# amolrpatil21/PorQua

Hardware: AMD Instinct MI355X
Metric: QPs solved/sec (rebalance dates) at N=1000 assets, 1-8 GPU; x vs host CPU (higher is better)
Workload: dtype f64; 1 GPU; config3: long-only min-variance (P=2*Pearson cov, budget + box [0,1]), daily rebalance; n_assets=1000, window=252, dates_per_gpu=4749, global_batch=4749, parallelism=dates-sharded x1

## Files before the change

include/porqua_hip.h:

```cpp
#ifndef PORQUA_HIP_H
#define PORQUA_HIP_H

#include <stdint.h>

#ifdef __cplusplus
extern "C" {
#endif

#define PQ_VERSION 100

#define PQ_UNSOLVED 0
#define PQ_SOLVED 1
#define PQ_SOLVED_INACCURATE 2
#define PQ_MAX_ITER 3
#define PQ_NEED_REFACTOR 4
#define PQ_PRIMAL_INFEASIBLE (-3)
#define PQ_DUAL_INFEASIBLE (-4)
#define PQ_NON_CONVEX (-5)

#define PQ_OUT_OBJ 0
#define PQ_OUT_PRIM 1
#define PQ_OUT_DUAL 2
#define PQ_OUT_GAP 3
#define PQ_OUT_RHO 4
// ... 15 lines not shown
  const double* lb;  const double* ub;  int64_t box_stride;
} pq_problem;

typedef struct pq_state {
  double* K;     int64_t K_stride;
  double* Dt;    int64_t Dt_stride;
  double* x;     double* Px;
  double* z;     double* y;
  int32_t m_ld, mg_pad;
  double* rho;
  int32_t* iters; int32_t* status; int32_t* info;
  double* out;
  double* work;  int64_t work_stride;
} pq_state;

typedef struct pq_settings {
  double rho0, rho0_rel, sigma, alpha, eps_abs, eps_rel, rho_min, rho_max, adapt_tol, eq_scale,
      delta, dual_tol;
  int32_t max_iter, adapt_interval, polish, polish_rounds, refine_iters;
  double polish_fix_rel;
  int32_t polish_inner;
  int32_t min_iter;
  double polish_release_rel;
} pq_settings;

typedef struct pq_lowrank {
  const double* panel; int64_t ldp;
  const int32_t* rows; const int32_t* tlen; int32_t tmax;
  const double* mu; int64_t mu_stride;
  const double* w_scale;
  const double* dg; int64_t dg_stride;
} pq_lowrank;

int pq_version(void);
const char* pq_last_error(void);

int pq_window_mean(const double* panel, int64_t ldp, int32_t n, const int32_t* rows,
                   const int32_t* tlen, int32_t tmax, int32_t batch, double* mu,
                   int64_t mu_stride, void* stream);

int pq_window_sumsq(const double* panel, int64_t ldp, int32_t n, const int32_t* rows,
                    const int32_t* tlen, int32_t tmax, int32_t batch, const double* mu,
                    int64_t mu_stride, double* out, int64_t out_stride, void* stream);

int pq_window_moments_grouped(const double* panel, int64_t ldp, int32_t n, const int32_t* gdates,
                              int32_t ngroups, const int32_t* urows, int32_t umax,
// ... 238 lines not shown
```

porqua_amd/_lib.py:

```python
from __future__ import annotations

import ctypes
import os

_HERE = os.path.dirname(os.path.abspath(__file__))
LIB_PATH = os.environ.get("PQ_LIB_PATH") or os.path.join(_HERE, "libporqua_hip.so")

c_int32 = ctypes.c_int32
c_int64 = ctypes.c_int64
c_dp = ctypes.c_void_p

PQ_UNSOLVED = 0
PQ_SOLVED = 1
PQ_SOLVED_INACCURATE = 2
PQ_MAX_ITER = 3
PQ_NEED_REFACTOR = 4
PQ_PRIMAL_INFEASIBLE = -3
PQ_DUAL_INFEASIBLE = -4
PQ_NON_CONVEX = -5

PQ_PCT_OK, PQ_PCT_EMPTY_BUCKET, PQ_PCT_NAN_SCORE = range(3)
PQ_PCT_MAX_N = 16384
PQ_PCT_MAX_BUCKETS = 256

PQ_RP_OK, PQ_RP_MAX_SWEEPS, PQ_RP_BAD_INPUT = range(3)
PQ_RP_TMAX = 1024

PQ_HRP_OK, PQ_HRP_BAD_INPUT = range(2)
PQ_HRP_NMAX = 1024
PQ_HRP_SINGLE, PQ_HRP_COMPLETE, PQ_HRP_AVERAGE, PQ_HRP_WEIGHTED, PQ_HRP_WARD = range(5)
HRP_METHODS = {"single": PQ_HRP_SINGLE, "complete": PQ_HRP_COMPLETE, "average": PQ_HRP_AVERAGE,
               "weighted": PQ_HRP_WEIGHTED, "ward": PQ_HRP_WARD}

PQ_PCA_TMAX = 1024
PQ_PCA_KMAX = 64
PQ_PCA_OK, PQ_PCA_BAD_INPUT = range(2)

PQ_PG_RECORD = 384
PQ_PG_PASS_SCRATCH = 123537
PQ_PG_PENDING, PQ_PG_DONE, PQ_PG_FALLBACK, PQ_PG_SKIP = range(4)
PQ_PG_STATE = 3
PQ_PG_K, PQ_PG_SC, PQ_PG_W = 0, 5, 320

PQ_OUT_OBJ, PQ_OUT_PRIM, PQ_OUT_DUAL, PQ_OUT_GAP, PQ_OUT_RHO, PQ_OUT_NFREE, PQ_OUT_ROUNDS = range(7)
PQ_OUT_FIELDS = 8


def work_doubles(ld: int, mg_pad: int) -> int:
    return (9 + mg_pad) * ld + 512


class PorquaHipError(RuntimeError):
    pass


class PQProblem(ctypes.Structure):
    _fields_ = [
        ("n", c_int32), ("ld", c_int32), ("batch", c_int32), ("mg", c_int32),
        ("P", c_dp), ("P_stride", c_int64),
        ("p_scale", c_dp), ("p_diag", c_dp),
        ("q", c_dp), ("q_stride", c_int64),
        ("Cg", c_dp), ("Cg_stride", c_int64),
        ("lg", c_dp), ("ug", c_dp), ("g_stride", c_int64),
        ("lb", c_dp), ("ub", c_dp), ("box_stride", c_int64),
    ]
# ... 6 lines not shown
        ("x", c_dp), ("Px", c_dp),
        ("z", c_dp), ("y", c_dp),
        ("m_ld", c_int32), ("mg_pad", c_int32),
        ("rho", c_dp),
        ("iters", c_dp), ("status", c_dp), ("info", c_dp),
        ("out", c_dp),
        ("work", c_dp), ("work_stride", c_int64),
    ]


class PQSettings(ctypes.Structure):
    _fields_ = [
        ("rho0", ctypes.c_double), ("rho0_rel", ctypes.c_double),
        ("sigma", ctypes.c_double), ("alpha", ctypes.c_double),
        ("eps_abs", ctypes.c_double), ("eps_rel", ctypes.c_double),
        ("rho_min", ctypes.c_double), ("rho_max", ctypes.c_double),
        ("adapt_tol", ctypes.c_double), ("eq_scale", ctypes.c_double),
        ("delta", ctypes.c_double), ("dual_tol", ctypes.c_double),
        ("max_iter", c_int32), ("adapt_interval", c_int32), ("polish", c_int32),
        ("polish_rounds", c_int32), ("refine_iters", c_int32),
        ("polish_fix_rel", ctypes.c_double),
        ("polish_inner", ctypes.c_int32), ("min_iter", ctypes.c_int32),
        ("polish_release_rel", ctypes.c_double),
    ]


class PQLowRank(ctypes.Structure):
    _fields_ = [
        ("panel", c_dp), ("ldp", c_int64),
        ("rows", c_dp), ("tlen", c_dp), ("tmax", c_int32),
        ("mu", c_dp), ("mu_stride", c_int64),
        ("w_scale", c_dp),
        ("dg", c_dp), ("dg_stride", c_int64),
    ]


class PQGcap(ctypes.Structure):
    _fields_ = [
        ("gdates", c_dp), ("ngroups", c_int32),
        ("urows", c_dp), ("ucnt", c_dp), ("uoff", c_dp), ("umax", c_int32),
        ("gidx", c_dp), ("grho", c_dp),
        ("M", c_dp), ("Minv", c_dp), ("k_ld", c_int32), ("M_stride", c_int64),
        ("aq", c_dp), ("aq_stride", c_int64),
        ("hinv", c_dp), ("ldh", c_int32),
        ("gmax", c_int32),
    ]
# ... 157 lines not shown
```

porqua_amd/csrc/admm.hip:

```cpp
#include "admm_dev.h"
#include "capi_util.h"

namespace pq {

constexpr int AT = 512;
constexpr int AW = AT / 64;

struct PhaseClock {
#ifdef PQ_PROFILE
  long long a[8];
  long long t;
  __device__ void init() {
    for (int i = 0; i < 8; ++i) a[i] = 0;
    t = wall_clock64();
  }
  __device__ void stamp(int k) {
    __syncthreads();
    if (threadIdx.x == 0) {
      const long long now = wall_clock64();
      a[k] += now - t;
      t = now;
    }
  }
  __device__ void flush(double* dst) {
// ... 453 lines not shown
      gz[t] = zg[t];
      gy[t] = yg[t];
    }
    if (t == 0) {
      st.iters[b] = it;
      st.status[b] = status;
      st.rho[b] = rho;
    }
  }
}

__global__ void k_init_state(pq_problem pb, pq_state st, const int32_t* idx, pq_settings s,
                             const double* dg, int64_t dg_stride, const double* w_scale) {
  const int b = idx ? idx[blockIdx.x] : (int)blockIdx.x;
  const int ld = pb.ld;
  for (int i = threadIdx.x; i < ld; i += blockDim.x) {
    st.x[(int64_t)b * ld + i] = 0.0;
    st.Px[(int64_t)b * ld + i] = 0.0;
  }
  for (int i = threadIdx.x; i < st.m_ld; i += blockDim.x) {
    st.z[(int64_t)b * st.m_ld + i] = 0.0;
    st.y[(int64_t)b * st.m_ld + i] = 0.0;
  }
  double rho0 = s.rho0;
  if (s.rho0_rel > 0.0) {
    __shared__ double red[16];
    const double* P = pb.P + (int64_t)b * pb.P_stride;
    const double ps = pb.p_scale ? pb.p_scale[b] : 1.0;
    const double pd = pb.p_diag ? pb.p_diag[b] : 0.0;
    double sdiag = 0.0;
    if (dg) {
      const double psw = ps * (w_scale ? w_scale[b] : 1.0);
      for (int i = threadIdx.x; i < pb.n; i += blockDim.x) sdiag += psw * dg[(int64_t)b * dg_stride + i] + pd;
    } else {
      for (int i = threadIdx.x; i < pb.n; i += blockDim.x) sdiag += ps * P[(int64_t)i * ld + i] + pd;
    }
    sdiag = block_sum(sdiag, red);
    const double md = sdiag / pb.n;
    rho0 = (md > 0.0 && isfinite(md)) ? fmin(fmax(s.rho0_rel * md, s.rho_min), s.rho_max) : s.rho0;
  }
  if (threadIdx.x == 0) {
    st.rho[b] = rho0;
    st.iters[b] = 0;
    st.status[b] = PQ_UNSOLVED;
    st.info[b] = 0;
    for (int k = 0; k < PQ_OUT_FIELDS; ++k)
      st.out[(int64_t)b * PQ_OUT_FIELDS + k] = (k == PQ_OUT_OBJ || k == PQ_OUT_PRIM || k == PQ_OUT_DUAL ||
                                                k == PQ_OUT_GAP) ? __builtin_nan("") : 0.0;
  }
}

}

extern "C" int pq_init_state(const pq_problem* pb, pq_state* st, const int32_t* idx, int32_t nidx,
                             const pq_settings* s, void* stream) {
  PQ_CHECK_ARG(pb && st && s, "pq_init_state: null argument");
  PQ_CHECK_ARG(st->x && st->Px && st->z && st->y && st->rho && st->iters && st->status &&
                   st->info && st->out, "pq_init_state: state buffers missing");
  PQ_CHECK_ARG(st->m_ld >= st->mg_pad + pb->ld && st->mg_pad >= pb->mg, "pq_init_state: bad m_ld / mg_pad");
  const int grid = idx ? nidx : pb->batch;
  if (grid <= 0) return 0;
  PQ_CHECK_ARG(pb->P || s->rho0_rel <= 0.0, "pq_init_state: rho0_rel > 0 needs P (pq_init_state_lr for the window form)");
// ... 81 lines not shown
```

porqua_amd/csrc/admm_gcap.hip:

```cpp
#include "admm_dev.h"
#include "chol_dev.h"
#include "capi_util.h"

namespace pq {

constexpr int CT = 256;
constexpr int CNW = CT / 64;
constexpr int CHW = CT / 32;
constexpr int CTP1 = 5;
constexpr int CTP2 = 6;
constexpr int CG_MAX = 16;
constexpr int CU_MAX = 320;
constexpr int CMG = 4;
constexpr int CMGW = 24;
constexpr int CNZ = 4;
constexpr int CP1_ROWS = 16 * CNW * CTP1;
constexpr int CK_MAX = CP1_ROWS + 4;
constexpr int CH_MAX = 64;

#ifdef PQ_PROFILE
#define CSTAMP(k)                                                 \
  do {                                                            \
    __syncthreads();                                              \
    if (threadIdx.x == 0) {                                       \
// ... 6 lines not shown
#define CSTAMP(k) do { } while (0)
#endif

struct GConst {
  double c, sqc, d, rho;
};
__device__ __forceinline__ GConst gconst(const pq_lowrank& lr, const pq_problem& pb, const pq_settings& s, int b,
                                         double rho) {
  GConst g;
  g.c = (pb.p_scale ? pb.p_scale[b] : 1.0) * (lr.w_scale ? lr.w_scale[b] : 1.0);
  g.sqc = sqrt(fmax(g.c, 0.0));
  const double pd = pb.p_diag ? pb.p_diag[b] : 0.0;
  const double rb = pb.lb ? row_rho(pb.lb[(int64_t)b * pb.box_stride], pb.ub[(int64_t)b * pb.box_stride], rho, s) : 0.0;
  g.d = s.sigma + pd + rb;
  g.rho = rho;
  return g;
}

__device__ __forceinline__ double band_at(const double* band, int64_t ldo, int ru, int rv) {
  if (ru < rv) { const int z = ru; ru = rv; rv = z; }
  return band[(int64_t)ru * ldo + (ru - rv)];
}

__global__ __launch_bounds__(256) void k_gcap_assemble(pq_lowrank lr, pq_problem pb, pq_gcap gc, pq_settings s,
                                                       const double* band, int64_t ldo, int r0, const double* pc,
                                                       int64_t ldpc, const double* cc) {
  __shared__ int s_w[CU_MAX];
  __shared__ double s_sr[CMGW];
  const int grp = blockIdx.x;
  const int d0 = gc.gdates[grp];
  const int U = gc.ucnt[grp], mg = pb.mg, k_ld = gc.k_ld;
  const int t = threadIdx.x, w = wave_id(), l = lane_id();
  for (int u = t; u < U; u += 256) s_w[u] = gc.urows[(int64_t)grp * gc.umax + u] - r0;
  const GConst g = gconst(lr, pb, s, d0, gc.grho[grp]);
  if (t < mg) s_sr[t] = sqrt(row_rho(pb.lg[t], pb.ug[t], g.rho, s));
  __syncthreads();
  const double a1 = g.c / g.d, a2 = g.sqc / g.d;
  double* M = gc.M + (int64_t)grp * gc.M_stride;
  for (int i = w; i < k_ld; i += 4) {
    const int jend = (i / TB + 1) * TB;
    const bool icg = i >= U && i < U + mg;
    for (int j = l; j < jend; j += 64) {
      double v = (i == j) ? 1.0 : 0.0;
      const bool jcg = j >= U && j < U + mg;
      if (i < U && j < U) v += a1 * band_at(band, ldo, s_w[i], s_w[j]);
      else if (icg && j < U) v += a2 * s_sr[i - U] * pc[(int64_t)s_w[j] * ldpc + (i - U)];
      else if (i < U && jcg) v += a2 * s_sr[j - U] * pc[(int64_t)s_w[i] * ldpc + (j - U)];
      else if (icg && jcg) v += s_sr[i - U] * s_sr[j - U] / g.d * cc[(i - U) * mg + (j - U)];
      M[(int64_t)i * k_ld + j] = v;
    }
  }
}

__device__ __forceinline__ void wave_lds_sync() {
  __builtin_amdgcn_fence(__ATOMIC_RELEASE, "wavefront");
  __builtin_amdgcn_wave_barrier();
  __builtin_amdgcn_fence(__ATOMIC_ACQUIRE, "wavefront");
}
__device__ __forceinline__ void c_transpose(const double (&X)[4], double (&Xt)[4], double* tile) {
  const int l = lane_id(), cc = l & 15, g4 = l >> 4;
#pragma unroll
  for (int q = 0; q < 4; ++q) tile[(g4 + 4 * q) * 17 + cc] = X[q];
  wave_lds_sync();
#pragma unroll
  for (int q = 0; q < 4; ++q) Xt[q] = tile[cc * 17 + g4 + 4 * q];
  wave_lds_sync();
}
__device__ __forceinline__ f64x4 c_xty(const double (&X)[4], const double (&Y)[4], f64x4 acc) {
#pragma unroll
  for (int q = 0; q < 4; ++q) acc = __builtin_amdgcn_mfma_f64_16x16x4f64(X[q], Y[q], acc, 0, 0, 0);
  return acc;
}
template <typename HF>
// ... 1086 lines not shown

static int gcap_check(const pq_lowrank* lr, const pq_problem* pb, const pq_gcap* gc, const char* who) {
  PQ_CHECK_ARG(lr && pb && gc, "%s: null argument", who);
  PQ_CHECK_ARG(gc->gdates && gc->urows && gc->ucnt && gc->uoff && gc->gidx && gc->grho && gc->ngroups > 0,
               "%s: group plan missing", who);
  PQ_CHECK_ARG(gc->umax > 0 && gc->umax <= pq::CU_MAX, "%s: umax must be in (0, %d]", who, pq::CU_MAX);
  PQ_CHECK_ARG(pb->mg >= 0 && pb->mg <= pq::CMGW && pb->Cg_stride == 0 && pb->g_stride == 0,
               "%s: needs shared general rows, mg <= %d", who, pq::CMGW);
  PQ_CHECK_ARG(gc->k_ld % 64 == 0 && gc->k_ld >= 64 && gc->k_ld <= 384,
               "%s: need 64 <= k_ld <= 384, a multiple of 64 (k_ld=%d)", who, gc->k_ld);
  PQ_CHECK_ARG(gc->gmax >= 0 && gc->gmax <= pq::CG_MAX * 2, "%s: gmax must be in [0, %d] (gmax=%d)", who,
               pq::CG_MAX * 2, gc->gmax);
  return 0;
}

static int gcap_nb(const pq_gcap* gc) { return gc->gmax > pq::CG_MAX ? 2 : 1; }

extern "C" int pq_gcap_assemble(const pq_lowrank* lr, const pq_problem* pb, const pq_gcap* gc,
                                const pq_settings* s, const double* band, int64_t ldo, int32_t r0,
                                const double* pc, int64_t ldpc, const double* cc, void* stream) {
  if (gcap_check(lr, pb, gc, "pq_gcap_assemble")) return -1;
  PQ_CHECK_ARG(s && band && gc->M, "pq_gcap_assemble: null argument");
  PQ_CHECK_ARG(pb->mg == 0 || (pc && cc), "pq_gcap_assemble: general rows need pc and cc");
  hipLaunchKernelGGL(pq::k_gcap_assemble, dim3(gc->ngroups), dim3(256), 0, (hipStream_t)stream, *lr, *pb, *gc, *s,
                     band, ldo, r0, pc, ldpc, cc);
  PQ_CHECK_LAUNCH("pq_gcap_assemble");
  return 0;
}

extern "C" int pq_gcap_prepare(const pq_lowrank* lr, const pq_problem* pb, pq_state* st, const pq_gcap* gc,
                               const pq_settings* s, const int32_t* idx, int32_t nidx, const double* band,
                               int64_t ldo, int32_t r0, const double* pc, int64_t ldpc, void* stream) {
  if (gcap_check(lr, pb, gc, "pq_gcap_prepare")) return -1;
  PQ_CHECK_ARG(st && s && band && gc->Minv && gc->aq && gc->hinv, "pq_gcap_prepare: null argument");
  PQ_CHECK_ARG(gc->aq_stride >= 2 * (int64_t)gc->k_ld && gc->ldh > 0 && gc->ldh <= pq::CH_MAX,
               "pq_gcap_prepare: aq needs 2 k_ld per date, ldh <= %d", pq::CH_MAX);
  PQ_CHECK_ARG(pb->mg == 0 || pc, "pq_gcap_prepare: general rows need pc");
  PQ_CHECK_ARG(gc->umax <= pq::CU_MAX && pb->mg <= pq::CMGW, "pq_gcap_prepare: union or general rows too many");
  const int grid = idx ? nidx : gc->ngroups;
  if (grid <= 0) return 0;
  static const int skip = [] {
    const char* e = getenv("PQ_PREP_SKIP");
    return e ? atoi(e) : 0;
  }();
  if (gcap_nb(gc) == 2)
    hipLaunchKernelGGL(pq::k_gcap_prep<2>, dim3(grid), dim3(pq::PT_PREP), 0, (hipStream_t)stream, *lr, *pb, *st, *gc,
                       *s, idx, band, ldo, r0, pc, ldpc, skip);
  else
// ... 56 lines not shown
```

porqua_amd/csrc/pg_record.h:

```cpp
#pragma once
#include "common.h"
#include "../../include/porqua_hip.h"

namespace pq {

constexpr int PGR = PQ_PG_RECORD;
enum : int {
  R_K = 0, R_MA = 1, R_NZB = 2, R_STATE = 3, R_ROUNDS = 4, R_SC = 5,
  R_FORMED = 6, R_REUSE = 7,
  R_ACT = 64, R_LAM = 128, R_DA = 192, R_SOL = 256, R_AL = 288,
  R_W = 320, R_NFX = 321, R_FIX = 324, R_FIXV = 332, R_FXL = 340,
  R_GFORM = 348,
  R_KB = 349,
  R_LIST = 352, R_CNT = 360
};
constexpr int PG_NBUCKET = 6;
constexpr int PG_BIGB = 5;
__device__ __forceinline__ unsigned long long pg_count(const double* rec, int bk) {
  return reinterpret_cast<const unsigned long long*>(rec + R_CNT)[bk];
}
__device__ __forceinline__ int pg_listed(const double* rec, int bk, int i) {
  return (int)rec[(int64_t)i * PGR + R_LIST + bk];
}
int resident_grid(const void* kernel, int block, int B);
__device__ __forceinline__ int pg_bucket(int kb) {
  return kb <= 48 ? 0 : kb <= 64 ? 1 : kb <= 80 ? 2 : kb <= 96 ? 3 : 4;
}
constexpr int PG_KMAX = 128;
constexpr int PG_KBIG = 256;
constexpr int PG_MGMAX = 32;
constexpr int PG_WMB = 8;
constexpr int PG_WG_MAX = 24;
static_assert(R_FXL + PG_WMB <= R_GFORM && R_KB < R_LIST && R_LIST + 6 <= R_CNT && R_CNT + 6 <= PQ_PG_RECORD,
              "PQ_PG_RECORD too small");

struct PGWork {
  double *xs, *xb, *g, *Px, *rF, *solx, *pxb, *U;
  int *Fl, *fl, *posF;
  __device__ __forceinline__ PGWork(const pq_state& st, int b, int ld) {
    double* W = st.work + (int64_t)b * st.work_stride;
    xs = W;
    xb = W + ld;
    g = W + 2 * (int64_t)ld;
    Px = W + 3 * (int64_t)ld;
    Fl = reinterpret_cast<int*>(W + 4 * (int64_t)ld);
    posF = Fl + ld;
    rF = W + 5 * (int64_t)ld;
    solx = W + 6 * (int64_t)ld;
    pxb = W + 7 * (int64_t)ld;
    U = W + 8 * (int64_t)ld;
    fl = reinterpret_cast<int*>(U + (int64_t)st.mg_pad * ld);
  }
};

__device__ __forceinline__ int pk(int r, int c) { return ((r * (r + 1)) >> 1) + c; }

// ... 7 lines not shown
```

porqua_amd/csrc/polish_g.hip:

```cpp
#include <cstdlib>
#include <mutex>

#include "polish_dev.h"
#include "capi_util.h"
#include "pg_record.h"

namespace pq {


__global__ __launch_bounds__(PT) void k_pg_init(pq_lowrank lr, pq_problem pb, pq_state st, double* rec,
                                                pq_settings s) {
  __shared__ double red[16];
  const int b = blockIdx.x;
  const int t = threadIdx.x;
  double* R = rec + (int64_t)b * PGR;
  const int st0 = st.status[b];
  if (st0 != PQ_SOLVED && st0 != PQ_MAX_ITER) {
    if (t == 0) R[R_STATE] = PQ_PG_SKIP;
    return;
  }
  const int n = pb.n, ld = pb.ld, mg = pb.mg;
  const double ps = pb.p_scale ? pb.p_scale[b] : 1.0;
  const double pd = pb.p_diag ? pb.p_diag[b] : 0.0;
  const double psw = ps * (lr.w_scale ? lr.w_scale[b] : 1.0);
// ... 48 lines not shown
  }
  if (t == 0) {
    R[R_STATE] = PQ_PG_PENDING;
    R[R_ROUNDS] = 0;
    R[R_SC] = sc;
    R[R_K] = nfree;
    R[R_NZB] = 0;
    R[R_W] = 0;
    R[R_FORMED] = 0;
    R[R_REUSE] = 0;
  }
#ifdef PQ_PROFILE
  if (t >= 8 && t < 32) R[t] = 0.0;
#endif
}

__global__ __launch_bounds__(PT) void k_pg_setup(pq_problem pb, pq_state st, double* rec, int kmax, int wide_ok,
                                                 int kbig) {
  __shared__ int wcnt[PW];
  __shared__ int s_al[PG_MGMAX + 1];
  __shared__ double red[16];
  const int b = blockIdx.x;
  double* R = rec + (int64_t)b * PGR;
  if (R[R_STATE] != PQ_PG_PENDING) return;
  const int n = pb.n, ld = pb.ld, mg = pb.mg;
  const int t = threadIdx.x, w = wave_id(), l = lane_id();
  const double* q = pb.q + (int64_t)b * pb.q_stride;
  const double* Cg = pb.Cg ? pb.Cg + (int64_t)b * pb.Cg_stride : nullptr;
  const double* lg = pb.lg ? pb.lg + (int64_t)b * pb.g_stride : nullptr;
  const double* ug = pb.ug ? pb.ug + (int64_t)b * pb.g_stride : nullptr;
  const bool has_box = pb.lb != nullptr;
  const double* lb = has_box ? pb.lb + (int64_t)b * pb.box_stride : nullptr;
  const double* ub = has_box ? pb.ub + (int64_t)b * pb.box_stride : nullptr;
  PGWork wk(st, b, ld);
  const int seg = ((n + PW * 64 - 1) / (PW * 64)) * 64;
  const int lo = w * seg, hi = min(n, lo + seg);
  int c = 0;
  for (int i0 = lo; i0 < hi; i0 += 4 * 64) {
    int fv[4];
#pragma unroll
    for (int u = 0; u < 4; ++u) {
      const int i = i0 + 64 * u + l;
      fv[u] = wk.fl[i < hi ? i : lo];
    }
#pragma unroll
    for (int u = 0; u < 4; ++u) c += __popcll(__ballot(i0 + 64 * u + l < hi && fv[u] == 0));
// ... 1744 lines not shown
  double sum = 0.0;
  for (int j0 = hl; j0 < n; j0 += 4 * PPT) {
    double av[4], bv[4];
#pragma unroll
    for (int u = 0; u < 4; ++u) {
      const int j = j0 + u * PPT, jc = j < n ? j : 0;
      av[u] = a[jc];
      bv[u] = b[jc];
    }
#pragma unroll
    for (int u = 0; u < 4; ++u)
      if (j0 + u * PPT < n) sum += av[u] * bv[u];
  }
  return sum;
}
template <int MODE>
__global__ __launch_bounds__(PPT) void k_pg_post(pq_lowrank lr, pq_problem pb, pq_state st, double* rec,
                                                pq_settings s, const int32_t* gdates, int ngroups,
                                                const double* scr) {
  const int b = blockIdx.x;
  double* R = rec + (int64_t)b * PGR;
  if (MODE == 0 && b == 0 && threadIdx.x < PG_NBUCKET)
    reinterpret_cast<unsigned long long*>(rec + R_CNT)[threadIdx.x] = 0ull;
  if (!(R[R_STATE] == PQ_PG_PENDING && (MODE == 1 || R[R_NZB] != 0.0))) return;
  int lo = 0, hi = ngroups;
  while (hi - lo > 1) {
    const int mid = (lo + hi) >> 1;
    if (gdates[mid] <= b) lo = mid; else hi = mid;
  }
  const int grp = lo, hg = b - gdates[grp];
  __shared__ double red[16];
  const int hl = threadIdx.x;
  const int n = pb.n, ld = pb.ld, mg = pb.mg;
  PGWork wk(st, b, ld);
  const double* mu = lr.mu ? lr.mu + (int64_t)b * lr.mu_stride : nullptr;
  const double su = scr[(int64_t)grp * QSCR + (int64_t)QS * (QU + 4) * QG + QS * QG + hg];
  const double wsc = lr.w_scale ? lr.w_scale[b] : 1.0;
  if (MODE == 0) {
    for (int i = hl; i < n; i += PPT) wk.pxb[i] = wsc * (wk.pxb[i] - (mu ? mu[i] * su : 0.0));
    return;
  }
  const double ps = pb.p_scale ? pb.p_scale[b] : 1.0;
  const double pd = pb.p_diag ? pb.p_diag[b] : 0.0;
  const double* q = pb.q + (int64_t)b * pb.q_stride;
  const double* Cg = pb.Cg ? pb.Cg + (int64_t)b * pb.Cg_stride : nullptr;
  const double* lg = pb.lg ? pb.lg + (int64_t)b * pb.g_stride : nullptr;
// ... 79 lines not shown
        const int a = (int)R[R_ACT + r];
        const double lam = lamof(r);
        if (a == 0 && sum > ug[r] + ptol * (1.0 + fabs(ug[r]))) { R[R_ACT + r] = 2; bad = 1; }
        else if (a == 0 && sum < lg[r] - ptol * (1.0 + fabs(lg[r]))) { R[R_ACT + r] = 1; bad = 1; }
        else if (a == 2 && lam < -dtol) { R[R_ACT + r] = 0; bad = 1; }
        else if (a == 1 && lam > dtol) { R[R_ACT + r] = 0; bad = 1; }
      } else if (fabs(sum - ug[r]) > 1e-10 * (1.0 + fabs(ug[r]))) {
        bad = 1;
      }
    }
  }
  bad = block_max((double)bad, red) > 0.5;
  if (soft > 0.0)
    for (int i = hl; i < n; i += PPT) {
      const int f = wk.fl[i];
      if (f >= 5) wk.fl[i] = bad ? 0 : f - 4;
    }
  if (vtx && hl == 0) {
    R[R_LAM + r0] = lam0;
    R[R_SOL] = lam0;
  }
  if (bad) {
    if (hl == 0 && R[R_ROUNDS] >= s.polish_rounds) R[R_STATE] = PQ_PG_FALLBACK;
    return;
  }
  double* sx = st.x + (int64_t)b * ld;
  double* sz = st.z + (int64_t)b * st.m_ld;
  double* sy = st.y + (int64_t)b * st.m_ld;
  double xpx = 0.0, qx = 0.0, pres = 0.0, dres = 0.0, gapb = 0.0;
  for (int i0 = hl; i0 < n; i0 += 4 * PPT) {
    double xv[4], pv[4], gv[4], qv[4], lbv[4], ubv[4];
    int fv[4];
#pragma unroll
    for (int j = 0; j < 4; ++j) {
      const int i = i0 + j * PPT, ic = i < n ? i : 0;
      xv[j] = wk.xs[ic];
      pv[j] = wk.Px[ic];
      gv[j] = wk.g[ic];
      qv[j] = q[ic];
      fv[j] = wk.fl[ic];
      lbv[j] = has_box ? lb[ic] : 0.0;
      ubv[j] = has_box ? ub[ic] : 0.0;
    }
#pragma unroll
    for (int j = 0; j < 4; ++j) {
      const int i = i0 + j * PPT;
// ... 258 lines not shown
```

porqua_amd/engine.py:

```python
from __future__ import annotations

import os
import ctypes
import dataclasses
from dataclasses import dataclass

import numpy as np
import torch

from . import _lib

F64 = torch.float64


def round_up(v: int, m: int) -> int:
    return ((int(v) + m - 1) // m) * m


def _ptr(t):
    return None if t is None else ctypes.c_void_p(t.data_ptr())


def _stream():
    return ctypes.c_void_p(torch.cuda.current_stream().cuda_stream)
# ... 38 lines not shown
    eps_grouped_percap: bool = False
    min_iter: int = 0
    polish_fix_rel: float = 0.1
    polish_inner: int = 1
    polish_release_rel: float = 0.0

    def to_c(self, **override) -> _lib.PQSettings:
        return _lib.PQSettings(**{**{k: getattr(self, k) for k in _C_SETTINGS}, **override})

    @classmethod
    def from_params(cls, params) -> "Settings":
        s = cls()
        if params:
            for f in dataclasses.fields(cls):
                for key in (f.name, "admm_" + f.name):
                    if key in params and params[key] is not None:
                        v, typ = params[key], type(getattr(s, f.name))
                        if typ is bool and isinstance(v, str):
                            v = v.strip().lower() not in ("0", "false", "no", "off", "")
                        setattr(s, f.name, typ(v))
        return s


_C_SETTINGS = tuple(c[0] for c in _lib.PQSettings._fields_ if c[0] in Settings.__dataclass_fields__)




class QPBatch:

    def __init__(self, n: int, batch: int, mg: int, device=None, shared_constraints=True,
                 has_box=True, P=None):
        self.device = device or default_device()
        self.n, self.batch, self.mg = int(n), int(batch), int(mg)
        self.ld = round_up(max(n, 1), 64)
        self.mg_pad = round_up(max(mg, 1), 8)
        ld, dev = self.ld, self.device
        self.P = P if P is not None else torch.zeros((batch, ld, ld), dtype=F64, device=dev)
        self.q = torch.zeros((batch, ld), dtype=F64, device=dev)
        self.p_scale = None
        self.p_diag = None
        nc = 1 if shared_constraints else batch
        self.shared = shared_constraints
        self.Cg = torch.zeros((nc, max(mg, 1), ld), dtype=F64, device=dev)
        self.lg = torch.full((nc, max(mg, 1)), -np.inf, dtype=F64, device=dev)
        self.ug = torch.full((nc, max(mg, 1)), np.inf, dtype=F64, device=dev)
        self.has_box = has_box
# ... 224 lines not shown
        run = (lambda: self.graphs.run(name, fn)) if self.graphs is not None else fn
        if self.sink is None:
            return run()
        e0 = torch.cuda.Event(enable_timing=True)
        e1 = torch.cuda.Event(enable_timing=True)
        e0.record()
        r = run()
        e1.record()
        self.sink.append((name, e0, e1))
        return r


def solve(qb: QPBatch, settings: Settings | None = None, ws: Workspace | None = None,
          max_rounds: int = 64, events: list | None = None) -> BatchResult:
    tl = _Timeline(events)
    lib = _lib.load()
    settings = settings or Settings()
    s = settings.to_c()
    ws = ws or Workspace(qb)
    pb = qb.c_struct()
    st = ws.c_struct()
    strm = _stream()
    P_, S_, SS = ctypes.byref(pb), ctypes.byref(st), ctypes.byref(s)
    _lib.check(lib.pq_init_state(P_, S_, None, 0, SS, strm), "pq_init_state")
    _rho_floor_q(qb, ws, settings)
    _lib.check(tl("factor", lambda: lib.pq_factor_batched(P_, S_, None, 0, SS, 1, strm)),
               "pq_factor_batched")
    cnt = {"refactors": 0, "launches": 0}

    def admm_rounds(idx, nidx, SSx):
        for _ in range(max_rounds):
            _lib.check(tl("admm", lambda: lib.pq_admm_batched(P_, S_, _ptr(idx), nidx, SSx,
                                                              int(s.max_iter), strm)),
                       "pq_admm_batched")
            cnt["launches"] += 1
            need = torch.nonzero(ws.status == _lib.PQ_NEED_REFACTOR).flatten().to(torch.int32)
            k = int(need.numel())
            if k == 0:
                break
            idx, nidx = need.contiguous(), k
            _lib.check(tl("factor", lambda: lib.pq_factor_batched(P_, S_, _ptr(idx), nidx, SSx, 1, strm)),
                       "pq_factor_batched")
            cnt["refactors"] += k

    admm_rounds(None, 0, SS)
    if s.polish:
        _lib.check(tl("polish", lambda: lib.pq_polish_batched(P_, S_, None, 0, SS, strm)),
                   "pq_polish_batched")
        rp = _repolish_set(ws, settings)
        if rp is not None:
            pidx, pn, s3 = rp
            _lib.check(tl("polish", lambda: lib.pq_polish_batched(P_, S_, _ptr(pidx), pn, ctypes.byref(s3), strm)),
                       "pq_polish_batched (refine)")
        retry = _retry_set(ws, settings)
        if retry is not None:
            idx, nidx, s2 = retry
            _lib.check(tl("factor", lambda: lib.pq_factor_batched(P_, S_, _ptr(idx), nidx, SS, 1, strm)),
                       "pq_factor_batched (retry)")
            admm_rounds(idx, nidx, ctypes.byref(s2))
            _lib.check(tl("polish", lambda: lib.pq_polish_batched(P_, S_, _ptr(idx), nidx, SS, strm)),
                       "pq_polish_batched (retry)")
    return _batch_result(qb, ws, refactors=cnt["refactors"], admm_launches=cnt["launches"])


def _batch_result(qb: "QPBatch", ws: "Workspace", **counts) -> BatchResult:
    n, mg = qb.n, qb.mg
    return BatchResult(x=ws.x[:, :n], y=ws.y[:, :mg], z_box=ws.y[:, ws.mg_pad:ws.mg_pad + n],
                       status=ws.status, iters=ws.iters, out=ws.out, **counts)


def _rho_floor_q(qb: "QPBatch", ws: "Workspace", settings: Settings):
    if settings.rho0_qrel > 0:
        qinf = qb.q[:, :qb.n].abs().amax(1)
        torch.clamp(torch.maximum(ws.rho, settings.rho0_qrel * qinf), settings.rho_min, settings.rho_max,
                    out=ws.rho)


def _repolish_set(ws: "Workspace", settings: Settings):
    if settings.refine_retry <= settings.refine_iters:
        return None
    bad = torch.nonzero(ws.status == _lib.PQ_SOLVED_INACCURATE).flatten().to(torch.int32)
    m = int(bad.numel())
    if m == 0:
        return None
    ws.status[bad.long()] = _lib.PQ_SOLVED
    return bad.contiguous(), m, settings.to_c(refine_iters=settings.refine_retry)


def _retry_set(ws: "Workspace", settings: Settings):
    bad = torch.nonzero(ws.status == _lib.PQ_SOLVED_INACCURATE).flatten().to(torch.int32)
    m = int(bad.numel())
    if m == 0 or settings.eps_retry <= 0 or settings.eps_retry >= min(settings.eps_abs, settings.eps_rel):
        return None
    ws.status[bad.long()] = _lib.PQ_UNSOLVED
    return bad.contiguous(), m, settings.to_c(eps_abs=settings.eps_retry, eps_rel=settings.eps_retry)


def _window_span(rows, tlen):
# ... 498 lines not shown

    def pg_round(self):
        _lib.check(self.lib.pq_polish_grouped_round(*self.pg["round"]), "pq_polish_grouped_round")
        self.pg["rounds"] += 1

    def pg_rounds_host(self):
        rec = self.pg["rec"]
        while self.pg["rounds"] < int(self.s.polish_rounds):
            if self.pg["rounds"] >= 2 and not bool((rec[:, _lib.PQ_PG_STATE] == _lib.PQ_PG_PENDING).any()):
                break
            self.pg_round()

    def polish_grouped(self):
        self.pg_start(True)
        self.pg_round()
        self.pg_rounds_host()
        self.pg_finish()

    def polish_sync_free(self):
        ws, rounds = self.ws, int(self.s.polish_rounds)
        self.pg_start(False)
        for _ in range(min(int(self.sf_rounds or rounds), rounds)):
            self.pg_round()
        st_pg = self.pg["rec"][:, _lib.PQ_PG_STATE]
        flag = ((st_pg == _lib.PQ_PG_PENDING) | (st_pg == _lib.PQ_PG_FALLBACK) |
                (ws.status == _lib.PQ_NEED_REFACTOR) | (ws.status == _lib.PQ_SOLVED_INACCURATE) |
                (ws.status == _lib.PQ_UNSOLVED)).any()
        if ws._sf_flag is None:
            ws._sf_flag = torch.zeros((), dtype=torch.bool, device=ws.device)
        ws._sf_flag.copy_(flag)
        return dict(self.pg)

    def pg_finish(self):
        ws = self.ws
        fb = torch.nonzero(self.pg["rec"][:, _lib.PQ_PG_STATE] == _lib.PQ_PG_FALLBACK).flatten().to(torch.int32)
        m = self.fallbacks = int(fb.numel())
        if m:
            ws.pg_fallback = fb
            if self.route.loose_eps > 0:
                ws.status[fb.long()] = _lib.PQ_UNSOLVED
                self.admm_rounds(fb.contiguous(), m, self.SS, name="admm (resume, inside polish)")
            sfb = self.settings.to_c(refine_iters=max(self.settings.refine_iters, 2))
            self.polish_w(fb.contiguous(), m, ctypes.byref(sfb), name="polish (fallback, inside polish)")

    def result(self) -> BatchResult:
        return _batch_result(self.qb, self.ws, refactors=self.refactors, admm_launches=self.launches,
                             polish_fallbacks=self.fallbacks, capacitance=self.route.capacitance)


def solve_lowrank(qb: QPBatch, lr: LowRank, settings: Settings | None = None,
                  ws: Workspace | None = None, max_rounds: int = 64, events: list | None = None,
                  polish: bool = True, groups: "GroupPlan | None" = None, band: bool = True,
                  fuse: bool = True, grouped_polish: bool = True, gcap: bool = True,
                  eig: "EigCap | None" = None, wide_polish: bool = True, sync_free: bool = False,
                  graphs: "StageGraphs | None" = None, sf_rounds: int | None = None,
                  host_work=None, sweep: "SweepPlan | None" = None) -> BatchResult:
    settings = settings or Settings()
    ws = ws or Workspace(qb, dense=False)
    if not lowrank_applicable(qb, lr):
        raise _lib.PorquaHipError(f"low-rank form not applicable (k={lr.tmax + qb.mg}, n={qb.n})")
    route = lowrank_route(qb, lr, ws, groups, settings, polish=polish, band=band, fuse=fuse,
                          grouped_polish=grouped_polish, gcap=gcap, wide_polish=wide_polish, sync_free=sync_free,
                          eig=eig, sweep=sweep)
    tl = _Timeline(events, graphs if route.sync_free else None)
    if tl.graphs is not None:
        tl.graphs.begin()
    c = _LowRankSolve(qb, lr, ws, settings, route, tl, groups, eig, sweep, wide_polish, max_rounds, sf_rounds)
    ws.gcap_groups = route.plan if route.admm == "gcap" else None
    ws.sweep_admm = sweep if route.admm == "sweep" else None
    ws.pg_fallback = None
    _lib.check(c.lib.pq_init_state_lr(*c.LPS, None, 0, c.SS, c.strm), "pq_init_state_lr")
    _rho_floor_q(qb, ws, settings)
    if band:
        c.bd = tl("gram", lambda: _band_setup(qb, lr, c.strm, w_min=route.band_wmin))
    ws.band_shape = (c.bd["nrows"], c.bd["W"]) if c.bd is not None else None
    if route.admm == "gcap":
        c.group_cap()
    tl("factor", lambda: c.refactor(None, 0, c.SS))

    SS_admm = c.SS
    if route.loose_eps > 0:
        sl = settings.to_c(eps_abs=route.loose_eps, eps_rel=route.loose_eps, min_iter=route.loose_min_iter)
        SS_admm = ctypes.byref(sl)
    c.admm_rounds(None, 0, SS_admm)

    if c.sync_free:
        c.pg = dict(tl("polish", c.polish_sync_free))
        if host_work is not None:
            host_work()
        if not bool(ws._sf_flag.item()):
            return c.result()
        if bool((ws.status == _lib.PQ_NEED_REFACTOR).any() | (ws.status == _lib.PQ_UNSOLVED).any()):
            return solve_lowrank(qb, lr, settings=settings, ws=ws, max_rounds=max_rounds, events=events,
                                 polish=polish, groups=groups, band=band, fuse=fuse, grouped_polish=grouped_polish,
                                 gcap=gcap, eig=eig, wide_polish=wide_polish)
# ... 91 lines not shown
        good = np.zeros(0, dtype=bool)
    joins = np.concatenate([[False], good])
    run_start = np.maximum.accumulate(np.where(~joins, np.arange(B), 0)) if B else np.zeros(0, np.int64)
    starts = np.flatnonzero((np.arange(B) - run_start) % max(int(group), 1) == 0)
    return np.concatenate([starts, [B]]).astype(np.int32), shift


class SlidePlan:

    def __init__(self, rows, tlen, device, group: int = 32, smax: int = 64):
        gs, sh = slide_plan(rows, tlen, group, smax)
        self.ngroups = len(gs) - 1
        self.gstart = torch.from_numpy(gs).to(device)
        self.shift = torch.from_numpy(sh).to(device)


GROUP_MAX_DATES = 16
GCAP_MAX_DATES = int(os.environ.get("PQ_GCAP_GMAX", "32"))
GCAP32_WIDE = os.environ.get("PQ_GCAP32_WIDE", "1") != "0"
GCAP_FACTOR = os.environ.get("PQ_GCAP_FACTOR", "batched")
GROUP_MAX_UNION = 320


SWEEP_ADMM = os.environ.get("PQ_SWEEP_ADMM", "1") != "0"


class SweepPlan:

    GMAX = 64

    def __init__(self, counts, device, q_shared: bool = False):
        self.q_shared = bool(q_shared)
        starts, b = [], 0
        for c in counts:
            starts.extend(range(b, b + int(c), self.GMAX))
            b += int(c)
        starts.append(b)
        self.gdates = torch.tensor(starts, dtype=torch.int32, device=device)
        self.ngroups = len(starts) - 1
        self.scratch = None

    def applicable(self, qb: "QPBatch", lr: "LowRank", k_ld: int) -> bool:
        return (SWEEP_ADMM and self.ngroups > 0 and lr.tmax <= 256 and k_ld <= 256 and qb.mg <= 4
                and qb.lb is not None and qb.ub is not None and qb.shared)

    def buffer(self, qb: "QPBatch", lib) -> torch.Tensor:
# ... 596 lines not shown
```

Measured before the change: 746,900 QPs/s.

## Fold rho floor and sync-free flag into kernels; tile gcap assembly

Moves the q-based rho0 floor out of separate torch ops and into the init-state kernel. Replaces the multi-op torch reduction for the sync-free fallback flag with a device-side flag written by the polish kernels. It also splits gcap M assembly into one block per lower-triangular 64x64 tile per group instead of one block per group. The aim is to cut small kernel launches and to raise parallelism in assembly, at the cost of extra flag-handling logic that must stay consistent with the host predicate.

Result: faster. 760,200 QPs/s, median of 6 (+1.8%).

```diff
diff --git a/include/porqua_hip.h b/include/porqua_hip.h
--- a/include/porqua_hip.h
+++ b/include/porqua_hip.h
@@ -61,6 +61,7 @@
   int32_t polish_inner;
   int32_t min_iter;
   double polish_release_rel;
+  double rho0_qrel;
 } pq_settings;
 
 typedef struct pq_lowrank {
diff --git a/porqua_amd/_lib.py b/porqua_amd/_lib.py
--- a/porqua_amd/_lib.py
+++ b/porqua_amd/_lib.py
@@ -41,6 +41,7 @@
 PQ_PG_PENDING, PQ_PG_DONE, PQ_PG_FALLBACK, PQ_PG_SKIP = range(4)
 PQ_PG_STATE = 3
 PQ_PG_K, PQ_PG_SC, PQ_PG_W = 0, 5, 320
+PQ_PG_SFLAG = 366
 
 PQ_OUT_OBJ, PQ_OUT_PRIM, PQ_OUT_DUAL, PQ_OUT_GAP, PQ_OUT_RHO, PQ_OUT_NFREE, PQ_OUT_ROUNDS = range(7)
 PQ_OUT_FIELDS = 8
@@ -93,6 +94,7 @@
         ("polish_fix_rel", ctypes.c_double),
         ("polish_inner", ctypes.c_int32), ("min_iter", ctypes.c_int32),
         ("polish_release_rel", ctypes.c_double),
+        ("rho0_qrel", ctypes.c_double),
     ]
 
 
diff --git a/porqua_amd/csrc/admm.hip b/porqua_amd/csrc/admm.hip
--- a/porqua_amd/csrc/admm.hip
+++ b/porqua_amd/csrc/admm.hip
@@ -499,9 +499,9 @@
     st.z[(int64_t)b * st.m_ld + i] = 0.0;
     st.y[(int64_t)b * st.m_ld + i] = 0.0;
   }
+  __shared__ double red[16];
   double rho0 = s.rho0;
   if (s.rho0_rel > 0.0) {
-    __shared__ double red[16];
     const double* P = pb.P + (int64_t)b * pb.P_stride;
     const double ps = pb.p_scale ? pb.p_scale[b] : 1.0;
     const double pd = pb.p_diag ? pb.p_diag[b] : 0.0;
@@ -515,6 +515,18 @@
     sdiag = block_sum(sdiag, red);
     const double md = sdiag / pb.n;
     rho0 = (md > 0.0 && isfinite(md)) ? fmin(fmax(s.rho0_rel * md, s.rho_min), s.rho_max) : s.rho0;
+  }
+  if (s.rho0_qrel > 0.0 && pb.q) {
+    const double* q = pb.q + (int64_t)b * pb.q_stride;
+    double qm = 0.0, qnan = 0.0;
+    for (int i = threadIdx.x; i < pb.n; i += blockDim.x) {
+      const double v = q[i];
+      qm = fmax(qm, fabs(v));
+      if (v != v) qnan = 1.0;
+    }
+    qm = block_max(qm, red);
+    qnan = block_max(qnan, red);
+    rho0 = qnan > 0.0 ? __builtin_nan("") : fmin(fmax(fmax(rho0, s.rho0_qrel * qm), s.rho_min), s.rho_max);
   }
   if (threadIdx.x == 0) {
     st.rho[b] = rho0;
diff --git a/porqua_amd/csrc/admm_gcap.hip b/porqua_amd/csrc/admm_gcap.hip
--- a/porqua_amd/csrc/admm_gcap.hip
+++ b/porqua_amd/csrc/admm_gcap.hip
@@ -52,9 +52,51 @@
   return band[(int64_t)ru * ldo + (ru - rv)];
 }
 
+__device__ __forceinline__ double gcap_m_elem(int i, int j, int U, int mg, const int* s_w, const double* s_sr,
+                                              double a1, double a2, double d, const double* band, int64_t ldo,
+                                              const double* pc, int64_t ldpc, const double* cc) {
+  double v = (i == j) ? 1.0 : 0.0;
+  const bool icg = i >= U && i < U + mg;
+  const bool jcg = j >= U && j < U + mg;
+  if (i < U && j < U) v += a1 * band_at(band, ldo, s_w[i], s_w[j]);
+  else if (icg && j < U) v += a2 * s_sr[i - U] * pc[(int64_t)s_w[j] * ldpc + (i - U)];
+  else if (i < U && jcg) v += a2 * s_sr[j - U] * pc[(int64_t)s_w[i] * ldpc + (j - U)];
+  else if (icg && jcg) v += s_sr[i - U] * s_sr[j - U] / d * cc[(i - U) * mg + (j - U)];
+  return v;
+}
+
 __global__ __launch_bounds__(256) void k_gcap_assemble(pq_lowrank lr, pq_problem pb, pq_gcap gc, pq_settings s,
                                                        const double* band, int64_t ldo, int r0, const double* pc,
                                                        int64_t ldpc, const double* cc) {
+  __shared__ int s_w[CU_MAX];
+  __shared__ double s_sr[CMGW];
+  const int k_ld = gc.k_ld, nb = k_ld / TB, nt = nb * (nb + 1) / 2;
+  const int grp = blockIdx.x / nt;
+  int rb = 0, cb = blockIdx.x - grp * nt;
+  while (cb > rb) cb -= ++rb;
+  const int d0 = gc.gdates[grp];
+  const int U = gc.ucnt[grp], mg = pb.mg;
+  const int t = threadIdx.x, w = wave_id(), l = lane_id();
+  if (t < 2 * TB) {
+    const int u = (t < TB ? rb * TB : cb * TB - TB) + t;
+    if (u < U) s_w[u] = gc.urows[(int64_t)grp * gc.umax + u] - r0;
+  }
+  const GConst g = gconst(lr, pb, s, d0, gc.grho[grp]);
+  if (t < mg) s_sr[t] = sqrt(row_rho(pb.lg[t], pb.ug[t], g.rho, s));
+  __syncthreads();
+  const double a1 = g.c / g.d, a2 = g.sqc / g.d;
+  double* M = gc.M + (int64_t)grp * gc.M_stride;
+  const int j = cb * TB + l;
+#pragma unroll 4
+  for (int r = 0; r < TB / 4; ++r) {
+    const int i = rb * TB + w + 4 * r;
+    M[(int64_t)i * k_ld + j] = gcap_m_elem(i, j, U, mg, s_w, s_sr, a1, a2, g.d, band, ldo, pc, ldpc, cc);
+  }
+}
+
+__global__ __launch_bounds__(256) void k_gcap_assemble_rows(pq_lowrank lr, pq_problem pb, pq_gcap gc, pq_settings s,
+                                                            const double* band, int64_t ldo, int r0,
+                                                            const double* pc, int64_t ldpc, const double* cc) {
   __shared__ int s_w[CU_MAX];
   __shared__ double s_sr[CMGW];
   const int grp = blockIdx.x;
@@ -69,16 +111,8 @@
   double* M = gc.M + (int64_t)grp * gc.M_stride;
   for (int i = w; i < k_ld; i += 4) {
     const int jend = (i / TB + 1) * TB;
-    const bool icg = i >= U && i < U + mg;
-    for (int j = l; j < jend; j += 64) {
-      double v = (i == j) ? 1.0 : 0.0;
-      const bool jcg = j >= U && j < U + mg;
-      if (i < U && j < U) v += a1 * band_at(band, ldo, s_w[i], s_w[j]);
-      else if (icg && j < U) v += a2 * s_sr[i - U] * pc[(int64_t)s_w[j] * ldpc + (i - U)];
-      else if (i < U && jcg) v += a2 * s_sr[j - U] * pc[(int64_t)s_w[i] * ldpc + (j - U)];
-      else if (icg && jcg) v += s_sr[i - U] * s_sr[j - U] / g.d * cc[(i - U) * mg + (j - U)];
-      M[(int64_t)i * k_ld + j] = v;
-    }
+    for (int j = l; j < jend; j += 64)
+      M[(int64_t)i * k_ld + j] = gcap_m_elem(i, j, U, mg, s_w, s_sr, a1, a2, g.d, band, ldo, pc, ldpc, cc);
   }
 }
 
@@ -1211,8 +1245,17 @@
   if (gcap_check(lr, pb, gc, "pq_gcap_assemble")) return -1;
   PQ_CHECK_ARG(s && band && gc->M, "pq_gcap_assemble: null argument");
   PQ_CHECK_ARG(pb->mg == 0 || (pc && cc), "pq_gcap_assemble: general rows need pc and cc");
-  hipLaunchKernelGGL(pq::k_gcap_assemble, dim3(gc->ngroups), dim3(256), 0, (hipStream_t)stream, *lr, *pb, *gc, *s,
-                     band, ldo, r0, pc, ldpc, cc);
+  static const int old_form = [] {
+    const char* e = getenv("PQ_GCAP_ASSEMBLE_OLD");
+    return e ? atoi(e) : 0;
+  }();
+  const int nb = gc->k_ld / 64;
+  if (old_form > 0)
+    hipLaunchKernelGGL(pq::k_gcap_assemble_rows, dim3(gc->ngroups), dim3(256), 0, (hipStream_t)stream, *lr, *pb, *gc,
+                       *s, band, ldo, r0, pc, ldpc, cc);
+  else
+    hipLaunchKernelGGL(pq::k_gcap_assemble, dim3(gc->ngroups * (nb * (nb + 1) / 2)), dim3(256), 0, (hipStream_t)stream,
+                       *lr, *pb, *gc, *s, band, ldo, r0, pc, ldpc, cc);
   PQ_CHECK_LAUNCH("pq_gcap_assemble");
   return 0;
 }
diff --git a/porqua_amd/csrc/pg_record.h b/porqua_amd/csrc/pg_record.h
--- a/porqua_amd/csrc/pg_record.h
+++ b/porqua_amd/csrc/pg_record.h
@@ -12,7 +12,8 @@
   R_W = 320, R_NFX = 321, R_FIX = 324, R_FIXV = 332, R_FXL = 340,
   R_GFORM = 348,
   R_KB = 349,
-  R_LIST = 352, R_CNT = 360
+  R_LIST = 352, R_CNT = 360,
+  R_SFLAG = 366
 };
 constexpr int PG_NBUCKET = 6;
 constexpr int PG_BIGB = 5;
@@ -31,7 +32,8 @@
 constexpr int PG_MGMAX = 32;
 constexpr int PG_WMB = 8;
 constexpr int PG_WG_MAX = 24;
-static_assert(R_FXL + PG_WMB <= R_GFORM && R_KB < R_LIST && R_LIST + 6 <= R_CNT && R_CNT + 6 <= PQ_PG_RECORD,
+static_assert(R_FXL + PG_WMB <= R_GFORM && R_KB < R_LIST && R_LIST + 6 <= R_CNT && R_CNT + 6 <= R_SFLAG &&
+                  R_SFLAG < PQ_PG_RECORD,
               "PQ_PG_RECORD too small");
 
 struct PGWork {
diff --git a/porqua_amd/csrc/polish_g.hip b/porqua_amd/csrc/polish_g.hip
--- a/porqua_amd/csrc/polish_g.hip
+++ b/porqua_amd/csrc/polish_g.hip
@@ -94,6 +94,7 @@
   __shared__ double red[16];
   const int b = blockIdx.x;
   double* R = rec + (int64_t)b * PGR;
+  if (b == 0 && threadIdx.x == 0) *reinterpret_cast<unsigned long long*>(rec + R_SFLAG) = 0ull;
   if (R[R_STATE] != PQ_PG_PENDING) return;
   const int n = pb.n, ld = pb.ld, mg = pb.mg;
   const int t = threadIdx.x, w = wave_id(), l = lane_id();
@@ -1884,6 +1885,12 @@
   double* R = rec + (int64_t)b * PGR;
   if (MODE == 0 && b == 0 && threadIdx.x < PG_NBUCKET)
     reinterpret_cast<unsigned long long*>(rec + R_CNT)[threadIdx.x] = 0ull;
+  auto left_for_host = [&]() { *reinterpret_cast<unsigned long long*>(rec + R_SFLAG) = 1ull; };
+  if (MODE == 1 && R[R_STATE] != PQ_PG_PENDING && threadIdx.x == 0) {
+    const int stt = st.status[b];
+    if (R[R_STATE] == PQ_PG_FALLBACK || stt == PQ_NEED_REFACTOR || stt == PQ_SOLVED_INACCURATE || stt == PQ_UNSOLVED)
+      left_for_host();
+  }
   if (!(R[R_STATE] == PQ_PG_PENDING && (MODE == 1 || R[R_NZB] != 0.0))) return;
   int lo = 0, hi = ngroups;
   while (hi - lo > 1) {
@@ -2009,6 +2016,7 @@
   }
   if (bad) {
     if (hl == 0 && R[R_ROUNDS] >= s.polish_rounds) R[R_STATE] = PQ_PG_FALLBACK;
+    if (hl == 0) left_for_host();
     return;
   }
   double* sx = st.x + (int64_t)b * ld;
diff --git a/porqua_amd/engine.py b/porqua_amd/engine.py
--- a/porqua_amd/engine.py
+++ b/porqua_amd/engine.py
@@ -84,7 +84,8 @@
         return s
 
 
-_C_SETTINGS = tuple(c[0] for c in _lib.PQSettings._fields_ if c[0] in Settings.__dataclass_fields__)
+_C_SETTINGS = tuple(c[0] for c in _lib.PQSettings._fields_
+                    if c[0] in Settings.__dataclass_fields__ and c[0] != "rho0_qrel")
 
 
 
@@ -355,8 +356,9 @@
     st = ws.c_struct()
     strm = _stream()
     P_, S_, SS = ctypes.byref(pb), ctypes.byref(st), ctypes.byref(s)
-    _lib.check(lib.pq_init_state(P_, S_, None, 0, SS, strm), "pq_init_state")
-    _rho_floor_q(qb, ws, settings)
+    s_init = _init_settings(settings)
+    _lib.check(lib.pq_init_state(P_, S_, None, 0, ctypes.byref(s_init), strm), "pq_init_state")
+    _rho_floor_q(qb, ws, settings, in_kernel=s_init.rho0_qrel > 0)
     _lib.check(tl("factor", lambda: lib.pq_factor_batched(P_, S_, None, 0, SS, 1, strm)),
                "pq_factor_batched")
     cnt = {"refactors": 0, "launches": 0}
@@ -402,11 +404,22 @@
                        status=ws.status, iters=ws.iters, out=ws.out, **counts)
 
 
-def _rho_floor_q(qb: "QPBatch", ws: "Workspace", settings: Settings):
-    if settings.rho0_qrel > 0:
+def _init_settings(settings: Settings) -> _lib.PQSettings:
+    return settings.to_c(rho0_qrel=0.0 if RHO_FLOOR_HOST else max(float(settings.rho0_qrel), 0.0))
+
+
+def _rho_floor_q(qb: "QPBatch", ws: "Workspace", settings: Settings, in_kernel: bool = False):
+    if settings.rho0_qrel > 0 and not in_kernel:
         qinf = qb.q[:, :qb.n].abs().amax(1)
         torch.clamp(torch.maximum(ws.rho, settings.rho0_qrel * qinf), settings.rho_min, settings.rho_max,
                     out=ws.rho)
+
+
+def sf_flag_torch(rec: torch.Tensor, status: torch.Tensor) -> torch.Tensor:
+    st_pg = rec[:, _lib.PQ_PG_STATE]
+    return ((st_pg == _lib.PQ_PG_PENDING) | (st_pg == _lib.PQ_PG_FALLBACK) |
+            (status == _lib.PQ_NEED_REFACTOR) | (status == _lib.PQ_SOLVED_INACCURATE) |
+            (status == _lib.PQ_UNSOLVED)).any()
 
 
 def _repolish_set(ws: "Workspace", settings: Settings):
@@ -951,13 +964,14 @@
         self.pg_start(False)
         for _ in range(min(int(self.sf_rounds or rounds), rounds)):
             self.pg_round()
-        st_pg = self.pg["rec"][:, _lib.PQ_PG_STATE]
-        flag = ((st_pg == _lib.PQ_PG_PENDING) | (st_pg == _lib.PQ_PG_FALLBACK) |
-                (ws.status == _lib.PQ_NEED_REFACTOR) | (ws.status == _lib.PQ_SOLVED_INACCURATE) |
-                (ws.status == _lib.PQ_UNSOLVED)).any()
         if ws._sf_flag is None:
             ws._sf_flag = torch.zeros((), dtype=torch.bool, device=ws.device)
-        ws._sf_flag.copy_(flag)
+        rec = self.pg["rec"]
+        if self.pg["rounds"] > 0 and not SF_FLAG_HOST:
+            left = rec[0, _lib.PQ_PG_SFLAG:_lib.PQ_PG_SFLAG + 1].view(torch.int64)[0]
+            torch.ne(left, 0, out=ws._sf_flag)
+        else:
+            ws._sf_flag.copy_(sf_flag_torch(rec, ws.status))
         return dict(self.pg)
 
     def pg_finish(self):
@@ -998,8 +1012,9 @@
     ws.gcap_groups = route.plan if route.admm == "gcap" else None
     ws.sweep_admm = sweep if route.admm == "sweep" else None
     ws.pg_fallback = None
-    _lib.check(c.lib.pq_init_state_lr(*c.LPS, None, 0, c.SS, c.strm), "pq_init_state_lr")
-    _rho_floor_q(qb, ws, settings)
+    s_init = _init_settings(settings)
+    _lib.check(c.lib.pq_init_state_lr(*c.LPS, None, 0, ctypes.byref(s_init), c.strm), "pq_init_state_lr")
+    _rho_floor_q(qb, ws, settings, in_kernel=s_init.rho0_qrel > 0)
     if band:
         c.bd = tl("gram", lambda: _band_setup(qb, lr, c.strm, w_min=route.band_wmin))
     ws.band_shape = (c.bd["nrows"], c.bd["W"]) if c.bd is not None else None
@@ -1137,6 +1152,8 @@
 GROUP_MAX_UNION = 320
 
 
+RHO_FLOOR_HOST = os.environ.get("PQ_RHO_FLOOR_HOST", "0") != "0"
+SF_FLAG_HOST = os.environ.get("PQ_SF_FLAG_HOST", "0") != "0"
 SWEEP_ADMM = os.environ.get("PQ_SWEEP_ADMM", "1") != "0"
 
 
```
